# ArthurBrussee/brush

Hardware: NVIDIA H100
Metric: fwd+bwd Mpix/s @1M Gaussians 1080p (higher is better)
Workload: dtype f32

## Files before the change

### brush_b200/csrc/blend_bwd.cu

```cuda
#include "blend_common.cuh"

namespace bg {

constexpr int BROW_ID = 12;
constexpr int BFACT = 12;

__device__ __forceinline__ float rcp_approx_f(float x) { float r; asm("rcp.approx.ftz.f32 %0, %1;" : "=f"(r) : "f"(x)); return r; }
__device__ __forceinline__ float sqrt_approx_f(float x) { float r; asm("sqrt.approx.ftz.f32 %0, %1;" : "=f"(r) : "f"(x)); return r; }

template <bool STATS, bool SMOOTH, bool DEPTH>
__global__ void __launch_bounds__(RASTER_THREADS)
blend_bwd_kernel(const float *__restrict__ projected, const uint32_t *__restrict__ cgid_from_isect,
                 const uint32_t *__restrict__ tile_offsets, const float4 *__restrict__ out_img,
                 const float4 *__restrict__ v_output, const uint32_t *__restrict__ live_masks,
                 const uint32_t *__restrict__ warp_batches, float *__restrict__ v_combined,
                 unsigned long long *__restrict__ stats, BlendUniforms u, const float *__restrict__ depths,
                 const float *__restrict__ out_depth, const float *__restrict__ v_depth, float *__restrict__ v_z) {
    __shared__ BlendStage s_stage[RASTER_WARPS];
    __shared__ __align__(16) float s_fact[RASTER_WARPS][2][WB * BFACT];

    const uint32_t tile = blockIdx.x;
    const uint32_t tid = threadIdx.x, lane = tid & 31u, wid = tid >> 5;
    const uint32_t num_batches = __ldg(warp_batches + tile * RASTER_WARPS + wid);
    BlendStage &st = s_stage[wid];
    if (lane == 0) { mbar_init(&st.bar[0], 1); mbar_init(&st.bar[1], 1); }
    __syncthreads();
    if (num_batches == 0) return;
    uint32_t phase_bits = 0u;
    const uint32_t range_lo = tile_offsets[tile * 2];
    const uint32_t tile_x0 = (tile % u.tiles_x) * TILE_W, tile_y0 = (tile / u.tiles_x) * TILE_W;
    const uint32_t blk_x0 = tile_x0 + 8u * (wid & 1u), blk_y0 = tile_y0 + 8u * (wid >> 1);
    const uint32_t pix_x = blk_x0 + (lane & 7u), pix_y0 = blk_y0 + (lane >> 3), pix_y1 = pix_y0 + 4u;
    const bool inside0 = pix_x < u.img_w && pix_y0 < u.img_h;
    const bool inside1 = pix_x < u.img_w && pix_y1 < u.img_h;
    const float px = (float)pix_x + 0.5f, py0 = (float)pix_y0 + 0.5f;
    const float2 npy2 = make_float2(-py0, -(py0 + 4.0f));
    const float img_wf = (float)u.img_w, img_hf = (float)u.img_h;
    const float hw = img_hf / img_wf, hw2 = hw * hw;

    float2 T2 = make_float2(0.0f, 0.0f);
    float2 rem_r = T2, rem_g = T2, rem_b = T2;
    float2 vo_r = T2, vo_g = T2, vo_b = T2, nvo_w = T2, ifa = T2;
    {
        auto load = [&](bool inside, uint32_t pix_y, float &T, float &rr, float &rg, float &rb, float &vr, float &vg,
                        float &vb, float &nvw, float &inv) {
            if (!inside) return;
            const size_t pix_id = (size_t)pix_x + (size_t)pix_y * u.img_w;
            const float4 o = __ldg(out_img + pix_id);
            const float4 vo = __ldg(v_output + pix_id);
            const float t_final = 1.0f - o.w;
            T = 1.0f;
            rr = o.x - t_final * u.bg_r; rg = o.y - t_final * u.bg_g; rb = o.z - t_final * u.bg_b;
            vr = vo.x; vg = vo.y; vb = vo.z;
            nvw = -((vo.w - (u.bg_r * vo.x + u.bg_g * vo.y + u.bg_b * vo.z)) * t_final);
            inv = img_wf / fmaxf(o.w, 1.0e-5f);
        };
        load(inside0, pix_y0, T2.x, rem_r.x, rem_g.x, rem_b.x, vo_r.x, vo_g.x, vo_b.x, nvo_w.x, ifa.x);
        load(inside1, pix_y1, T2.y, rem_r.y, rem_g.y, rem_b.y, vo_r.y, vo_g.y, vo_b.y, nvo_w.y, ifa.y);
    }
    float2 rem_d = make_float2(0.0f, 0.0f), vo_d = rem_d;
    if constexpr (DEPTH) {
        const size_t pix0 = (size_t)pix_x + (size_t)pix_y0 * u.img_w, pix1 = (size_t)pix_x + (size_t)pix_y1 * u.img_w;
        if (inside0) { rem_d.x = __ldg(out_depth + pix0); vo_d.x = __ldg(v_depth + pix0); }
        if (inside1) { rem_d.y = __ldg(out_depth + pix1); vo_d.y = __ldg(v_depth + pix1); }
    }

    constexpr int NS = DEPTH ? 12 : 10, NH = NS / 2;
    const bool b4 = lane & 16u, b3 = lane & 8u, b2 = lane & 4u, b1 = lane & 2u;
    const uint32_t idx5 = (b3 ? 3u : 0u) + (b2 ? 2u : 0u) + (b1 ? 1u : 0u);
    const uint32_t slot = (b4 ? (uint32_t)NH : 0u) + idx5;
    const bool owner = !(lane & 1u) && !(b2 && b1) && (DEPTH ? slot != 11u : !(b3 && b2));
    const uint32_t lt_mask = (1u << lane) - 1u;

    const size_t mbase = blend_mask_base(range_lo, tile) + wid;
    auto load_mask = [&](uint32_t b) -> uint32_t {
        return b < num_batches ? __ldg(live_masks + mbase + (size_t)b * RASTER_WARPS) : 0u;
    };
    float z_next = 0.0f;
    auto stage = [&](uint32_t b, uint32_t m) -> uint32_t {
        uint32_t id = 0;
        const uint32_t n = (uint32_t)__popc(m);
        if (n == 0) return 0u;
        if ((m >> lane) & 1u) {
            id = __ldg(cgid_from_isect + range_lo + b * WB + lane);
            st.ids[b & 1u][__popc(m & lt_mask)] = id;
            if constexpr (DEPTH) z_next = __ldg(depths + id);
        }
        stage_rows_tma(st, b & 1u, n, projected, lane);
        return id;
    };
    unsigned long long st_iter = 0, st_blend = 0, st_stop = 0;
    uint32_t m_cur = load_mask(0), m_next = load_mask(1);
    uint32_t id_next = stage(0, m_cur);
    for (uint32_t b = 0; b < num_batches; b++) {
        const uint32_t m = m_cur, my_id = id_next;
        const float my_z = z_next;
        m_cur = m_next;
        m_next = load_mask(b + 2);
        id_next = stage(b + 1, m_cur);
        const uint32_t n = (uint32_t)__popc(m);
        if (n == 0) continue;
        mbar_wait(&st.bar[b & 1u], (phase_bits >> (b & 1u)) & 1u);
        phase_bits ^= 1u << (b & 1u);
        float *rows = st.rows[b & 1u];
        float *fact = s_fact[wid][b & 1u];
        if ((m >> lane) & 1u) {
            const uint32_t slot_r = (uint32_t)__popc(m & lt_mask);
            float *mine = rows + slot_r * ROW;
            const float4 B = *reinterpret_cast<const float4 *>(mine + 4);
            const float bcol = mine[8];
            *reinterpret_cast<float4 *>(mine + 4) = make_float4(B.x, -B.y, fmaxf(B.z, 0.0f), fmaxf(B.w, 0.0f));
            mine[8] = fmaxf(bcol, 0.0f);
            mine[BROW_ID] = __uint_as_float(my_id);
            float *f = fact + slot_r * BFACT;
            *reinterpret_cast<float4 *>(f) = make_float4(-1.0f, -1.0f, -0.5f, -1.0f);
            *reinterpret_cast<float4 *>(f + 4) =
                make_float4(-0.5f, B.z >= 0.0f ? -1.0f : 0.0f, B.w >= 0.0f ? -1.0f : 0.0f, bcol >= 0.0f ? -1.0f : 0.0f);
            *reinterpret_cast<float2 *>(f + 8) = make_float2(1.0f / B.y, 1.0f);
            if constexpr (DEPTH) {
                mine[ROW_Z] = my_z;
                *reinterpret_cast<float2 *>(f + 10) = make_float2(-1.0f, 0.0f);
            }
        }
        __syncwarp();
        if (STATS) st_iter += n;
        for (uint32_t j = 0; j < n; j++) {
            const float *row = rows + j * ROW;
            const float4 A = *reinterpret_cast<const float4 *>(row);
            const float4 B = *reinterpret_cast<const float4 *>(row + 4);
            const float4 C = *reinterpret_cast<const float4 *>(row + 8);
            const float dx = A.x - px;
            float2 dy2;
            const float2 sg = pair_sigma(dx, A.y, C.y, C.z, C.w, npy2, dy2);
            const float2 gs = make_float2(ex2_approx(-sg.x), ex2_approx(-sg.y));
            const float2 noa = fmul2_rn(gs, bcast2(B.y));
            const float2 nal = make_float2(fmaxf(-0.999f, noa.x), fmaxf(-0.999f, noa.y));
            float2 nae = nal;
            bool act0, act1;
            if constexpr (SMOOTH) {
                const float2 ae = smooth_alpha(make_float2(-nal.x, -nal.y), sg, act0, act1);
                nae = make_float2(-ae.x, -ae.y);
            } else {
                act0 = sg.x >= 0.0f && noa.x <= -ALPHA_CUTOFF_MID; act1 = sg.y >= 0.0f && noa.y <= -ALPHA_CUTOFF_MID;
            }
            const float2 oma = fadd2_rn(nae, bcast2(1.0f));
            const float2 nT = fmul2_rn(T2, oma);
            const bool c0 = act0 && nT.x > 1.0e-4f, c1 = act1 && nT.y > 1.0e-4f;
            if (STATS) {
                st_blend += __popc(__ballot_sync(0xffffffffu, c0)) + __popc(__ballot_sync(0xffffffffu, c1));
                st_stop += __popc(__ballot_sync(0xffffffffu, act0 && !c0 && T2.x > 1.0e-4f)) +
                           __popc(__ballot_sync(0xffffffffu, act1 && !c1 && T2.y > 1.0e-4f));
            }
            const float2 nalc = make_float2(c0 ? nae.x : 0.0f, c1 ? nae.y : 0.0f);
            const float2 nals = make_float2((c0 && noa.x >= -0.999f) ? nal.x : 0.0f, (c1 && noa.y >= -0.999f) ? nal.y : 0.0f);
            const float2 ra = make_float2(rcp_approx_f(oma.x), rcp_approx_f(oma.y));
            const float2 nvis = fmul2_rn(nalc, T2);
            const float2 G5 = fmul2_rn(nvis, vo_r), G6 = fmul2_rn(nvis, vo_g), G7 = fmul2_rn(nvis, vo_b);
            const float2 u_r = ffma2_rn(T2, bcast2(-B.z), rem_r);
            const float2 u_g = ffma2_rn(T2, bcast2(-B.w), rem_g);
            const float2 u_b = ffma2_rn(T2, bcast2(-C.x), rem_b);
            float2 nd = fmul2_rn(u_r, vo_r);
            nd = ffma2_rn(u_g, vo_g, nd);
            nd = ffma2_rn(u_b, vo_b, nd);
            float z = 0.0f;
            if constexpr (DEPTH) {
                z = row[ROW_Z];
                const float2 u_d = ffma2_rn(T2, bcast2(-z), rem_d);
                nd = ffma2_rn(u_d, vo_d, nd);
            }
            float2 nva = fmul2_rn(fadd2_rn(nd, nvo_w), ra);
            if constexpr (SMOOTH) nva = fmul2_rn(nva, make_float2(smooth_alpha_deriv(-nal.x), smooth_alpha_deriv(-nal.y)));
            const float2 nvs = fmul2_rn(nals, nva);
            const float2 vsx = fmul2_rn(nvs, bcast2(dx)), vsy = fmul2_rn(nvs, dy2);
            const float2 G0 = ffma2_rn(bcast2(A.z), vsx, fmul2_rn(bcast2(A.w), vsy));
            const float2 G1 = ffma2_rn(bcast2(A.w), vsx, fmul2_rn(bcast2(B.x), vsy));
            const float2 G2 = fmul2_rn(vsx, bcast2(dx)), G3 = fmul2_rn(vsx, dy2), G4 = fmul2_rn(vsy, dy2);
            const float2 nn = ffma2_rn(G0, G0, fmul2_rn(fmul2_rn(G1, bcast2(hw2)), G1));
            const float2 G9 = fmul2_rn(make_float2(sqrt_approx_f(nn.x), sqrt_approx_f(nn.y)), ifa);
            rem_r = ffma2_rn(nvis, bcast2(B.z), rem_r);
            rem_g = ffma2_rn(nvis, bcast2(B.w), rem_g);
            rem_b = ffma2_rn(nvis, bcast2(C.x), rem_b);
            float2 G10 = make_float2(0.0f, 0.0f);
            if constexpr (DEPTH) {
                G10 = fmul2_rn(nvis, vo_d);
                rem_d = ffma2_rn(nvis, bcast2(z), rem_d);
            }
            T2.x = act0 ? nT.x : T2.x;
            T2.y = act1 ? nT.y : T2.y;
            float g[NS];
            g[0] = G0.x + G0.y; g[1] = G1.x + G1.y; g[2] = G2.x + G2.y; g[3] = G3.x + G3.y; g[4] = G4.x + G4.y;
            g[5] = G5.x + G5.y; g[6] = G6.x + G6.y; g[7] = G7.x + G7.y; g[8] = nvs.x + nvs.y; g[9] = G9.x + G9.y;
            if constexpr (DEPTH) { g[10] = G10.x + G10.y; g[11] = 0.0f; }
            float a5[6];
#pragma unroll
            for (int i = 0; i < NH; i++) {
                float send = b4 ? g[i] : g[i + NH];
                float keep = b4 ? g[i + NH] : g[i];
                a5[i] = keep + __shfl_xor_sync(0xffffffffu, send, 16);
            }
            if constexpr (!DEPTH) a5[5] = 0.0f;
            float b3v[4];
#pragma unroll
            for (int i = 0; i < 3; i++) {
                float send = b3 ? a5[i] : a5[i + 3];
                float keep = b3 ? a5[i + 3] : a5[i];
                b3v[i] = keep + __shfl_xor_sync(0xffffffffu, send, 8);
            }
            b3v[3] = 0.0f;
            float c2[2];
#pragma unroll
            for (int i = 0; i < 2; i++) {
                float send = b2 ? b3v[i] : b3v[i + 2];
                float keep = b2 ? b3v[i + 2] : b3v[i];
                c2[i] = keep + __shfl_xor_sync(0xffffffffu, send, 4);
            }
            float d1;
            {
                float send = b1 ? c2[0] : c2[1];
                float keep = b1 ? c2[1] : c2[0];
                d1 = keep + __shfl_xor_sync(0xffffffffu, send, 2);
            }
            d1 += __shfl_xor_sync(0xffffffffu, d1, 1);
            if (owner && d1 != 0.0f) {
                const uint32_t id = __float_as_uint(row[BROW_ID]);
                if (DEPTH && slot == 10u) atomicAdd(v_z + id, d1 * fact[j * BFACT + slot]);
                else atomicAdd(v_combined + (size_t)id * BG_VCOMBINED_STRIDE + slot, d1 * fact[j * BFACT + slot]);
            }
        }
        __syncwarp();
    }
    if (STATS && lane == 0) {
        atomicAdd(stats + 0, st_iter); atomicAdd(stats + 1, st_blend); atomicAdd(stats + 2, st_stop);
    }
}

cudaError_t launch_blend_bwd(cudaStream_t s, bool smooth, uint32_t num_tiles, const float *projected, const uint32_t *cgid_from_isect,
                             const uint32_t *tile_offsets, const float *out_img, const float *v_output, const uint32_t *live_masks,
                             const uint32_t *warp_batches, float *v_combined, unsigned long long *stats, uint32_t tiles_x,
                             uint32_t w, uint32_t h, const float *bg, const float *depths, const float *out_depth,
                             const float *v_depth, float *v_z) {
    BlendUniforms u;
    u.tiles_x = tiles_x; u.img_w = w; u.img_h = h; u.bg_r = bg[0]; u.bg_g = bg[1]; u.bg_b = bg[2];
#define BG_LAUNCH_BWD(ST, S, D, STATS_PTR)                                                                                \
    blend_bwd_kernel<ST, S, D><<<num_tiles, RASTER_THREADS, 0, s>>>(projected, cgid_from_isect, tile_offsets, (const float4 *)out_img, \
                                                                    (const float4 *)v_output, live_masks, warp_batches, v_combined, \
                                                                    STATS_PTR, u, depths, out_depth, v_depth, v_z)
    if (v_z) {
        if (smooth) BG_LAUNCH_BWD(false, true, true, nullptr);
        else BG_LAUNCH_BWD(false, false, true, nullptr);
    } else if (smooth) {
        BG_LAUNCH_BWD(false, true, false, nullptr);
    } else if (stats) {
        BG_LAUNCH_BWD(true, false, false, stats);
    } else {
        BG_LAUNCH_BWD(false, false, false, nullptr);
    }
#undef BG_LAUNCH_BWD
    return cudaGetLastError();
}

}
```

### brush_b200/csrc/blend_common.cuh

```cuda
#pragma once
#include "bg_common.cuh"

namespace bg {

constexpr int RASTER_WARPS = 4;
constexpr int RASTER_THREADS = RASTER_WARPS * 32;
constexpr int WB = 32;
constexpr int ROW = BG_PROJECTED_STRIDE;
constexpr int ROW_PT = 12;
constexpr int ROW_Z = 13;

struct BlendUniforms {
    uint32_t tiles_x, img_w, img_h;
    float bg_r, bg_g, bg_b;
};

__device__ __forceinline__ float2 bcast2(float a) { return make_float2(a, a); }

__device__ __forceinline__ size_t blend_mask_base(uint32_t range_lo, uint32_t tile) {
    return ((size_t)(range_lo >> 5) + tile) * RASTER_WARPS;
}

struct __align__(128) BlendStage {
    float rows[2][WB * ROW];
    uint32_t ids[2][WB];
    unsigned long long bar[2];
};

__device__ __forceinline__ void stage_rows_tma(BlendStage &st, uint32_t buf, uint32_t count, const float *projected, uint32_t lane) {
    asm volatile("fence.proxy.async.shared::cta;" ::: "memory");
    __syncwarp();
    if (lane == 0 && count > 0) {
        mbar_expect_tx(&st.bar[buf], count * (ROW * 4u));
        for (uint32_t r = 0; r < count; r++)
            tma_bulk_g2s(&st.rows[buf][r * ROW], projected + (size_t)st.ids[buf][r] * ROW, ROW * 4u, &st.bar[buf]);
    }
}

__device__ __forceinline__ bool block_may_hit(float mx, float my, float a, float b, float c, float thr, float x0,
                                              float x1, float y0, float y1) {
    if (!(a > 0.0f && c > 0.0f && a * c > b * b)) return true;
    const float xc = fminf(fmaxf(mx, x0), x1);
    const float yc = fminf(fmaxf(my, y0), y1);
    const bool out_x = xc != mx, out_y = yc != my;
    if (!(out_x || out_y)) return true;
    float best = 3.0e38f, err = 0.0f;
    if (out_x) {
        float dx = xc - mx;
        float ys = fminf(fmaxf(my - (b / c) * dx, y0), y1);
        float dy = ys - my;
        float t0 = a * dx * dx, t1 = c * dy * dy, t2 = b * dx * dy;
        float s = 0.5f * (t0 + t1) + t2;
        if (s < best) { best = s; err = fabsf(t0) + fabsf(t1) + 2.0f * fabsf(t2); }
    }
    if (out_y) {
        float dy = yc - my;
        float xs = fminf(fmaxf(mx - (b / a) * dy, x0), x1);
        float dx = xs - mx;
        float t0 = a * dx * dx, t1 = c * dy * dy, t2 = b * dx * dy;
        float s = 0.5f * (t0 + t1) + t2;
        if (s < best) { best = s; err = fabsf(t0) + fabsf(t1) + 2.0f * fabsf(t2); }
    }
    return !(best > thr + 0.05f + 4.0e-6f * err);
}

__device__ __forceinline__ float ex2_approx(float x) { float r; asm("ex2.approx.ftz.f32 %0, %1;" : "=f"(r) : "f"(x)); return r; }

__device__ __forceinline__ float2 pair_sigma(float dx, float my, float cy, float cz, float cw, float2 npy2, float2 &dy2) {
    const float hx = __fmul_rn(__fmul_rn(cz, dx), dx);
    const float bdx = __fmul_rn(cw, dx);
    dy2 = fadd2_rn(bcast2(my), npy2);
    float2 t = fmul2_rn(bcast2(cy), dy2);
    t = ffma2_rn(t, dy2, bcast2(hx));
    return ffma2_rn(bcast2(bdx), dy2, t);
}

__device__ __forceinline__ float cutoff_weight(float alpha) {
    const float lo = ALPHA_CUTOFF_MID - 0.5f * ALPHA_CUTOFF_BAND;
    const float t = fminf(fmaxf(__fdiv_rn(__fsub_rn(alpha, lo), ALPHA_CUTOFF_BAND), 0.0f), 1.0f);
    return __fmul_rn(__fmul_rn(t, t), __fmaf_rn(-2.0f, t, 3.0f));
}
__device__ __forceinline__ float cutoff_weight_deriv(float alpha) {
    const float low = ALPHA_CUTOFF_MID - 0.5f * ALPHA_CUTOFF_BAND, high = ALPHA_CUTOFF_MID + 0.5f * ALPHA_CUTOFF_BAND;
    bool inside = alpha > low && alpha < high;
    float t = (alpha - low) / ALPHA_CUTOFF_BAND;
    return inside ? (6.0f * t - 6.0f * t * t) / ALPHA_CUTOFF_BAND : 0.0f;
}
constexpr float SMOOTH_THR_EXTRA = 0.1365f;

__device__ __forceinline__ float2 smooth_alpha(float2 alpha, float2 sg, bool &act0, bool &act1) {
    const float2 w = make_float2(cutoff_weight(alpha.x), cutoff_weight(alpha.y));
    act0 = sg.x >= 0.0f && w.x > 0.0f;
    act1 = sg.y >= 0.0f && w.y > 0.0f;
    return fmul2_rn(alpha, w);
}
__device__ __forceinline__ float smooth_alpha_deriv(float alpha) {
    return fmaf(alpha, cutoff_weight_deriv(alpha), cutoff_weight(alpha));
}

}
```

### brush_b200/csrc/blend_fwd.cu

```cuda
#include "blend_common.cuh"

namespace bg {

template <bool BWD_INFO, bool SMOOTH, bool DEPTH>
__global__ void __launch_bounds__(RASTER_THREADS)
blend_fwd_kernel(const float *__restrict__ projected, const uint32_t *__restrict__ cgid_from_isect,
                 uint32_t *__restrict__ tile_offsets, const uint32_t *__restrict__ gid_from_cgid,
                 float4 *__restrict__ out_f32, uint32_t *__restrict__ out_packed, float *__restrict__ visible,
                 uint32_t *__restrict__ live_masks, uint32_t *__restrict__ warp_batches, BlendUniforms u,
                 const float *__restrict__ depths, float *__restrict__ out_depth) {
    __shared__ BlendStage s_stage[RASTER_WARPS];
    __shared__ uint32_t s_max_useful;

    const uint32_t tile = blockIdx.x;
    const uint32_t tid = threadIdx.x, lane = tid & 31u, wid = tid >> 5;
    const uint32_t tile_x0 = (tile % u.tiles_x) * TILE_W, tile_y0 = (tile / u.tiles_x) * TILE_W;
    const uint32_t blk_x0 = tile_x0 + 8u * (wid & 1u), blk_y0 = tile_y0 + 8u * (wid >> 1);
    const uint32_t pix_x = blk_x0 + (lane & 7u), pix_y0 = blk_y0 + (lane >> 3), pix_y1 = pix_y0 + 4u;
    const bool inside0 = pix_x < u.img_w && pix_y0 < u.img_h;
    const bool inside1 = pix_x < u.img_w && pix_y1 < u.img_h;
    const float px = (float)pix_x + 0.5f, py0 = (float)pix_y0 + 0.5f;
    const float2 npy2 = make_float2(-py0, -(py0 + 4.0f));
    const float rx0 = (float)blk_x0 + 0.5f, rx1 = rx0 + 7.0f, ry0 = (float)blk_y0 + 0.5f, ry1 = ry0 + 7.0f;

    const uint32_t range_lo = tile_offsets[tile * 2], range_hi = tile_offsets[tile * 2 + 1];
    if (BWD_INFO && tid == 0) s_max_useful = range_lo;
    BlendStage &st = s_stage[wid];
    if (lane == 0) { mbar_init(&st.bar[0], 1); mbar_init(&st.bar[1], 1); }
    __syncthreads();
    uint32_t phase_bits = 0u;

    float2 T2 = make_float2(1.0f, 1.0f);
    float2 Tt2 = make_float2(inside0 ? 1.0f : 0.0f, inside1 ? 1.0f : 0.0f);
    float2 r2 = make_float2(0.0f, 0.0f), g2 = r2, b2 = r2, d2 = r2;
    uint32_t last_useful = range_lo;

    const uint32_t num_batches = (range_hi - range_lo + WB - 1) / WB;
    const size_t mbase = blend_mask_base(range_lo, tile) + wid;
    uint32_t batches_walked = 0;
    uint32_t next_id = 0;
    float next_z = 0.0f;
    auto prefetch = [&](uint32_t b) {
        const uint32_t start = range_lo + b * WB;
        const uint32_t count = min((uint32_t)WB, range_hi - start);
        const uint32_t id = lane < count ? __ldg(cgid_from_isect + start + lane) : 0u;
        next_id = id;
        if constexpr (DEPTH) next_z = lane < count ? __ldg(depths + id) : 0.0f;
        if (lane < count) st.ids[b & 1u][lane] = id;
        stage_rows_tma(st, b & 1u, count, projected, lane);
    };
    if (num_batches > 0 && __any_sync(0xffffffffu, inside0 || inside1)) {
        prefetch(0);
        for (uint32_t b = 0; b < num_batches; b++) {
            const uint32_t batch_start = range_lo + b * WB;
            const uint32_t count = min((uint32_t)WB, range_hi - batch_start);
            const uint32_t my_id = next_id;
            const float my_z = next_z;
            if (b + 1 < num_batches) prefetch(b + 1);
            mbar_wait(&st.bar[b & 1u], (phase_bits >> (b & 1u)) & 1u);
            phase_bits ^= 1u << (b & 1u);
            float *rows = st.rows[b & 1u];
            bool hit = false;
            if (lane < count) {
                float *mine = rows + lane * ROW;
                const float4 A = *reinterpret_cast<const float4 *>(mine);
                const float4 B = *reinterpret_cast<const float4 *>(mine + 4);
                const float bcol = mine[8];
                float pt = mine[ROW_PT];
                if constexpr (SMOOTH) pt += SMOOTH_THR_EXTRA;
                hit = block_may_hit(A.x, A.y, A.z, A.w, B.x, pt, rx0, rx1, ry0, ry1);
                *reinterpret_cast<float2 *>(mine + 6) = make_float2(fmaxf(B.z, 0.0f), fmaxf(B.w, 0.0f));
                mine[8] = fmaxf(bcol, 0.0f);
                if constexpr (DEPTH) mine[ROW_Z] = my_z;
            }
            uint32_t bits = __ballot_sync(0xffffffffu, hit);
            uint32_t used_m = 0, acted_m = 0;
            while (bits) {
                const uint32_t s = (uint32_t)__ffs(bits) - 1u;
                bits &= bits - 1u;
                const float *row = rows + s * ROW;
                const float4 A = *reinterpret_cast<const float4 *>(row);
                const float4 B = *reinterpret_cast<const float4 *>(row + 4);
                const float4 C = *reinterpret_cast<const float4 *>(row + 8);
                float2 dy2;
                const float2 sg = pair_sigma(A.x - px, A.y, C.y, C.z, C.w, npy2, dy2);
                const float2 gs = make_float2(ex2_approx(-sg.x), ex2_approx(-sg.y));
                const float2 oa = fmul2_rn(gs, bcast2(B.y));
                float a0 = fminf(0.999f, oa.x), a1 = fminf(0.999f, oa.y);
                bool act0, act1;
                if constexpr (SMOOTH) {
                    const float2 ae = smooth_alpha(make_float2(a0, a1), sg, act0, act1);
                    a0 = ae.x; a1 = ae.y;
                } else {
                    act0 = sg.x >= 0.0f && oa.x >= ALPHA_CUTOFF_MID; act1 = sg.y >= 0.0f && oa.y >= ALPHA_CUTOFF_MID;
                }
                const float2 nT = fmul2_rn(Tt2, fadd2_rn(make_float2(-a0, -a1), bcast2(1.0f)));
                const bool c0 = act0 && nT.x > 1.0e-4f, c1 = act1 && nT.y > 1.0e-4f;
                const float2 vis = fmul2_rn(make_float2(c0 ? a0 : 0.0f, c1 ? a1 : 0.0f), T2);
                r2 = ffma2_rn(bcast2(B.z), vis, r2);
                g2 = ffma2_rn(bcast2(B.w), vis, g2);
                b2 = ffma2_rn(bcast2(C.x), vis, b2);
                if constexpr (DEPTH) d2 = ffma2_rn(bcast2(row[ROW_Z]), vis, d2);
                const uint32_t bit = 1u << s;
                const bool acted = (Tt2.x > 1.0e-4f && act0) || (Tt2.y > 1.0e-4f && act1);
                if (c0 || c1) used_m |= bit;
                if (BWD_INFO && acted) acted_m |= bit;
                T2.x = c0 ? nT.x : T2.x;
                T2.y = c1 ? nT.y : T2.y;
                Tt2.x = act0 ? nT.x : Tt2.x;
                Tt2.y = act1 ? nT.y : Tt2.y;
            }
            const uint32_t used = __reduce_or_sync(0xffffffffu, used_m);
            if (BWD_INFO) {
                const uint32_t acted = __reduce_or_sync(0xffffffffu, acted_m);
                if (lane == 0) live_masks[mbase + (size_t)b * RASTER_WARPS] = acted;
                if ((used >> lane) & 1u) {
                    visible[__ldg(gid_from_cgid + my_id)] = 1.0f;
                    last_useful = batch_start + lane + 1;
                }
            }
            batches_walked = b + 1;
            if (__all_sync(0xffffffffu, !(Tt2.x > 1.0e-4f) && !(Tt2.y > 1.0e-4f))) {
                if (b + 1 < num_batches) mbar_wait(&st.bar[(b + 1) & 1u], (phase_bits >> ((b + 1) & 1u)) & 1u);
                break;
            }
            __syncwarp();
        }
    }

    auto write_pixel = [&](float T, float r, float g, float bl, float d, uint32_t pix_y) {
        const float fr = r + T * u.bg_r, fg = g + T * u.bg_g, fb = bl + T * u.bg_b, fa = 1.0f - T;
        const size_t pix_id = (size_t)pix_x + (size_t)pix_y * u.img_w;
        if (BWD_INFO) {
            out_f32[pix_id] = make_float4(fr, fg, fb, fa);
            if constexpr (DEPTH) out_depth[pix_id] = d;
        } else {
            uint32_t r8 = (uint32_t)fminf(fmaxf(fr * 255.0f, 0.0f), 255.0f);
            uint32_t g8 = (uint32_t)fminf(fmaxf(fg * 255.0f, 0.0f), 255.0f);
            uint32_t b8 = (uint32_t)fminf(fmaxf(fb * 255.0f, 0.0f), 255.0f);
            uint32_t a8 = (uint32_t)fminf(fmaxf(fa * 255.0f, 0.0f), 255.0f);
            out_packed[pix_id] = r8 | (g8 << 8) | (b8 << 16) | (a8 << 24);
        }
    };
    if (inside0) write_pixel(T2.x, r2.x, g2.x, b2.x, d2.x, pix_y0);
    if (inside1) write_pixel(T2.y, r2.y, g2.y, b2.y, d2.y, pix_y1);
    if (BWD_INFO) {
        if (lane == 0) warp_batches[tile * RASTER_WARPS + wid] = batches_walked;
        uint32_t m = last_useful;
        for (int o = 16; o > 0; o >>= 1) m = max(m, __shfl_xor_sync(0xffffffffu, m, o));
        __syncthreads();
        if (lane == 0 && m > range_lo) atomicMax(&s_max_useful, m);
        __syncthreads();
        if (tid == 0) tile_offsets[tile * 2 + 1] = s_max_useful;
    }
}

cudaError_t launch_blend_fwd(cudaStream_t s, bool bwd_info, bool smooth, uint32_t num_tiles, const float *projected,
                             const uint32_t *cgid_from_isect, uint32_t *tile_offsets, const uint32_t *gid_from_cgid, void *out_img,
                             float *visible, uint32_t *live_masks, uint32_t *warp_batches, uint32_t tiles_x, uint32_t w,
                             uint32_t h, const float *bg, const float *depths, float *out_depth) {
    BlendUniforms u;
    u.tiles_x = tiles_x; u.img_w = w; u.img_h = h; u.bg_r = bg[0]; u.bg_g = bg[1]; u.bg_b = bg[2];
#define BG_LAUNCH_FWD(B, S, D, F32, PACKED, LM, WBAT)                                                                    \
    blend_fwd_kernel<B, S, D><<<num_tiles, RASTER_THREADS, 0, s>>>(projected, cgid_from_isect, tile_offsets, gid_from_cgid, \
                                                                   F32, PACKED, visible, LM, WBAT, u, depths, out_depth)
    if (!bwd_info)
        BG_LAUNCH_FWD(false, false, false, nullptr, (uint32_t *)out_img, nullptr, nullptr);
    else if (out_depth && !smooth)
        BG_LAUNCH_FWD(true, false, true, (float4 *)out_img, nullptr, live_masks, warp_batches);
    else if (out_depth)
        BG_LAUNCH_FWD(true, true, true, (float4 *)out_img, nullptr, live_masks, warp_batches);
    else if (!smooth)
        BG_LAUNCH_FWD(true, false, false, (float4 *)out_img, nullptr, live_masks, warp_batches);
    else
        BG_LAUNCH_FWD(true, true, false, (float4 *)out_img, nullptr, live_masks, warp_batches);
#undef BG_LAUNCH_FWD
    return cudaGetLastError();
}

}
```

Measured before the change: 1049.

## Cull splats before TMA staging in forward blend and compact staged rows

The forward blend prefetch now reads each candidate's conic and threshold straight from global memory and runs the block-hit test before staging. Only splats that may hit the block are bulk-copied into shared memory, in compacted order, and the blend loop walks them densely. Used and acted masks are remapped from compact slots back to lane bits with a ballot. This cuts TMA traffic and shared-memory use for culled splats, at the cost of extra global loads per lane during prefetch and extra ballot work. The staging helper is also shared with the backward kernel.

```diff
diff --git a/brush_b200/csrc/blend_bwd.cu b/brush_b200/csrc/blend_bwd.cu
--- a/brush_b200/csrc/blend_bwd.cu
+++ b/brush_b200/csrc/blend_bwd.cu
@@ -79,14 +79,11 @@
     float z_next = 0.0f;
     auto stage = [&](uint32_t b, uint32_t m) -> uint32_t {
         uint32_t id = 0;
-        const uint32_t n = (uint32_t)__popc(m);
-        if (n == 0) return 0u;
         if ((m >> lane) & 1u) {
             id = __ldg(cgid_from_isect + range_lo + b * WB + lane);
-            st.ids[b & 1u][__popc(m & lt_mask)] = id;
             if constexpr (DEPTH) z_next = __ldg(depths + id);
         }
-        stage_rows_tma(st, b & 1u, n, projected, lane);
+        stage_rows_compact(st, b & 1u, m, id, projected, lane);
         return id;
     };
     unsigned long long st_iter = 0, st_blend = 0, st_stop = 0;
diff --git a/brush_b200/csrc/blend_common.cuh b/brush_b200/csrc/blend_common.cuh
--- a/brush_b200/csrc/blend_common.cuh
+++ b/brush_b200/csrc/blend_common.cuh
@@ -35,6 +35,17 @@
         for (uint32_t r = 0; r < count; r++)
             tma_bulk_g2s(&st.rows[buf][r * ROW], projected + (size_t)st.ids[buf][r] * ROW, ROW * 4u, &st.bar[buf]);
     }
+}
+
+__device__ __forceinline__ uint32_t compact_slot(uint32_t m, uint32_t lane) { return (uint32_t)__popc(m & ((1u << lane) - 1u)); }
+
+__device__ __forceinline__ uint32_t stage_rows_compact(BlendStage &st, uint32_t buf, uint32_t m, uint32_t id,
+                                                       const float *projected, uint32_t lane) {
+    const uint32_t n = (uint32_t)__popc(m);
+    if (n == 0) return 0u;
+    if ((m >> lane) & 1u) st.ids[buf][compact_slot(m, lane)] = id;
+    stage_rows_tma(st, buf, n, projected, lane);
+    return n;
 }
 
 __device__ __forceinline__ bool block_may_hit(float mx, float my, float a, float b, float c, float thr, float x0,
diff --git a/brush_b200/csrc/blend_fwd.cu b/brush_b200/csrc/blend_fwd.cu
--- a/brush_b200/csrc/blend_fwd.cu
+++ b/brush_b200/csrc/blend_fwd.cu
@@ -38,81 +38,93 @@
     const uint32_t num_batches = (range_hi - range_lo + WB - 1) / WB;
     const size_t mbase = blend_mask_base(range_lo, tile) + wid;
     uint32_t batches_walked = 0;
-    uint32_t next_id = 0;
+    uint32_t next_id = 0, next_m = 0;
     float next_z = 0.0f;
     auto prefetch = [&](uint32_t b) {
         const uint32_t start = range_lo + b * WB;
-        const uint32_t count = min((uint32_t)WB, range_hi - start);
-        const uint32_t id = lane < count ? __ldg(cgid_from_isect + start + lane) : 0u;
+        const bool in = lane < min((uint32_t)WB, range_hi - start);
+        const uint32_t id = in ? __ldg(cgid_from_isect + start + lane) : 0u;
+        bool cand = false;
+        if (in) {
+            const float4 *row = reinterpret_cast<const float4 *>(projected + (size_t)id * ROW);
+            const float4 A = __ldg(row);
+            const float c = __ldg(projected + (size_t)id * ROW + 4);
+            float pt = __ldg(projected + (size_t)id * ROW + ROW_PT);
+            if constexpr (SMOOTH) pt += SMOOTH_THR_EXTRA;
+            cand = block_may_hit(A.x, A.y, A.z, A.w, c, pt, rx0, rx1, ry0, ry1);
+        }
         next_id = id;
-        if constexpr (DEPTH) next_z = lane < count ? __ldg(depths + id) : 0.0f;
-        if (lane < count) st.ids[b & 1u][lane] = id;
-        stage_rows_tma(st, b & 1u, count, projected, lane);
+        next_m = __ballot_sync(0xffffffffu, cand);
+        if constexpr (DEPTH) next_z = cand ? __ldg(depths + id) : 0.0f;
+        stage_rows_compact(st, b & 1u, next_m, id, projected, lane);
     };
     if (num_batches > 0 && __any_sync(0xffffffffu, inside0 || inside1)) {
         prefetch(0);
         for (uint32_t b = 0; b < num_batches; b++) {
             const uint32_t batch_start = range_lo + b * WB;
-            const uint32_t count = min((uint32_t)WB, range_hi - batch_start);
-            const uint32_t my_id = next_id;
+            const uint32_t m = next_m, my_id = next_id;
             const float my_z = next_z;
+            const uint32_t n = (uint32_t)__popc(m);
             if (b + 1 < num_batches) prefetch(b + 1);
-            mbar_wait(&st.bar[b & 1u], (phase_bits >> (b & 1u)) & 1u);
-            phase_bits ^= 1u << (b & 1u);
-            float *rows = st.rows[b & 1u];
-            bool hit = false;
-            if (lane < count) {
-                float *mine = rows + lane * ROW;
-                const float4 A = *reinterpret_cast<const float4 *>(mine);
-                const float4 B = *reinterpret_cast<const float4 *>(mine + 4);
-                const float bcol = mine[8];
-                float pt = mine[ROW_PT];
-                if constexpr (SMOOTH) pt += SMOOTH_THR_EXTRA;
-                hit = block_may_hit(A.x, A.y, A.z, A.w, B.x, pt, rx0, rx1, ry0, ry1);
-                *reinterpret_cast<float2 *>(mine + 6) = make_float2(fmaxf(B.z, 0.0f), fmaxf(B.w, 0.0f));
-                mine[8] = fmaxf(bcol, 0.0f);
-                if constexpr (DEPTH) mine[ROW_Z] = my_z;
+            else next_m = 0u;
+            uint32_t used = 0, acted = 0;
+            if (n > 0) {
+                mbar_wait(&st.bar[b & 1u], (phase_bits >> (b & 1u)) & 1u);
+                phase_bits ^= 1u << (b & 1u);
+                float *rows = st.rows[b & 1u];
+                if ((m >> lane) & 1u) {
+                    float *mine = rows + compact_slot(m, lane) * ROW;
+                    const float4 B = *reinterpret_cast<const float4 *>(mine + 4);
+                    const float bcol = mine[8];
+                    *reinterpret_cast<float2 *>(mine + 6) = make_float2(fmaxf(B.z, 0.0f), fmaxf(B.w, 0.0f));
+                    mine[8] = fmaxf(bcol, 0.0f);
+                    if constexpr (DEPTH) mine[ROW_Z] = my_z;
+                }
+                __syncwarp();
+                uint32_t used_m = 0, acted_m = 0;
+                for (uint32_t j = 0; j < n; j++) {
+                    const float *row = rows + j * ROW;
+                    const float4 A = *reinterpret_cast<const float4 *>(row);
+                    const float4 B = *reinterpret_cast<const float4 *>(row + 4);
+                    const float4 C = *reinterpret_cast<const float4 *>(row + 8);
+                    float2 dy2;
+                    const float2 sg = pair_sigma(A.x - px, A.y, C.y, C.z, C.w, npy2, dy2);
+                    const float2 gs = make_float2(ex2_approx(-sg.x), ex2_approx(-sg.y));
+                    const float2 oa = fmul2_rn(gs, bcast2(B.y));
+                    float a0 = fminf(0.999f, oa.x), a1 = fminf(0.999f, oa.y);
+                    bool act0, act1;
+                    if constexpr (SMOOTH) {
+                        const float2 ae = smooth_alpha(make_float2(a0, a1), sg, act0, act1);
+                        a0 = ae.x; a1 = ae.y;
+                    } else {
+                        act0 = sg.x >= 0.0f && oa.x >= ALPHA_CUTOFF_MID; act1 = sg.y >= 0.0f && oa.y >= ALPHA_CUTOFF_MID;
+                    }
+                    const float2 nT = fmul2_rn(Tt2, fadd2_rn(make_float2(-a0, -a1), bcast2(1.0f)));
+                    const bool c0 = act0 && nT.x > 1.0e-4f, c1 = act1 && nT.y > 1.0e-4f;
+                    const float2 vis = fmul2_rn(make_float2(c0 ? a0 : 0.0f, c1 ? a1 : 0.0f), T2);
+                    r2 = ffma2_rn(bcast2(B.z), vis, r2);
+                    g2 = ffma2_rn(bcast2(B.w), vis, g2);
+                    b2 = ffma2_rn(bcast2(C.x), vis, b2);
+                    if constexpr (DEPTH) d2 = ffma2_rn(bcast2(row[ROW_Z]), vis, d2);
+                    const uint32_t bit = 1u << j;
+                    const bool acts = (Tt2.x > 1.0e-4f && act0) || (Tt2.y > 1.0e-4f && act1);
+                    if (c0 || c1) used_m |= bit;
+                    if (BWD_INFO && acts) acted_m |= bit;
+                    T2.x = c0 ? nT.x : T2.x;
+                    T2.y = c1 ? nT.y : T2.y;
+                    Tt2.x = act0 ? nT.x : Tt2.x;
+                    Tt2.y = act1 ? nT.y : Tt2.y;
+                }
+                const bool cand = (m >> lane) & 1u;
+                const uint32_t slot = compact_slot(m, lane);
+                const uint32_t used_c = __reduce_or_sync(0xffffffffu, used_m);
+                used = __ballot_sync(0xffffffffu, cand && ((used_c >> slot) & 1u));
+                if (BWD_INFO) {
+                    const uint32_t acted_c = __reduce_or_sync(0xffffffffu, acted_m);
+                    acted = __ballot_sync(0xffffffffu, cand && ((acted_c >> slot) & 1u));
+                }
             }
-            uint32_t bits = __ballot_sync(0xffffffffu, hit);
-            uint32_t used_m = 0, acted_m = 0;
-            while (bits) {
-                const uint32_t s = (uint32_t)__ffs(bits) - 1u;
-                bits &= bits - 1u;
-                const float *row = rows + s * ROW;
-                const float4 A = *reinterpret_cast<const float4 *>(row);
-                const float4 B = *reinterpret_cast<const float4 *>(row + 4);
-                const float4 C = *reinterpret_cast<const float4 *>(row + 8);
-                float2 dy2;
-                const float2 sg = pair_sigma(A.x - px, A.y, C.y, C.z, C.w, npy2, dy2);
-                const float2 gs = make_float2(ex2_approx(-sg.x), ex2_approx(-sg.y));
-                const float2 oa = fmul2_rn(gs, bcast2(B.y));
-                float a0 = fminf(0.999f, oa.x), a1 = fminf(0.999f, oa.y);
-                bool act0, act1;
-                if constexpr (SMOOTH) {
-                    const float2 ae = smooth_alpha(make_float2(a0, a1), sg, act0, act1);
-                    a0 = ae.x; a1 = ae.y;
-                } else {
-                    act0 = sg.x >= 0.0f && oa.x >= ALPHA_CUTOFF_MID; act1 = sg.y >= 0.0f && oa.y >= ALPHA_CUTOFF_MID;
-                }
-                const float2 nT = fmul2_rn(Tt2, fadd2_rn(make_float2(-a0, -a1), bcast2(1.0f)));
-                const bool c0 = act0 && nT.x > 1.0e-4f, c1 = act1 && nT.y > 1.0e-4f;
-                const float2 vis = fmul2_rn(make_float2(c0 ? a0 : 0.0f, c1 ? a1 : 0.0f), T2);
-                r2 = ffma2_rn(bcast2(B.z), vis, r2);
-                g2 = ffma2_rn(bcast2(B.w), vis, g2);
-                b2 = ffma2_rn(bcast2(C.x), vis, b2);
-                if constexpr (DEPTH) d2 = ffma2_rn(bcast2(row[ROW_Z]), vis, d2);
-                const uint32_t bit = 1u << s;
-                const bool acted = (Tt2.x > 1.0e-4f && act0) || (Tt2.y > 1.0e-4f && act1);
-                if (c0 || c1) used_m |= bit;
-                if (BWD_INFO && acted) acted_m |= bit;
-                T2.x = c0 ? nT.x : T2.x;
-                T2.y = c1 ? nT.y : T2.y;
-                Tt2.x = act0 ? nT.x : Tt2.x;
-                Tt2.y = act1 ? nT.y : Tt2.y;
-            }
-            const uint32_t used = __reduce_or_sync(0xffffffffu, used_m);
             if (BWD_INFO) {
-                const uint32_t acted = __reduce_or_sync(0xffffffffu, acted_m);
                 if (lane == 0) live_masks[mbase + (size_t)b * RASTER_WARPS] = acted;
                 if ((used >> lane) & 1u) {
                     visible[__ldg(gid_from_cgid + my_id)] = 1.0f;
@@ -120,8 +132,8 @@
                 }
             }
             batches_walked = b + 1;
-            if (__all_sync(0xffffffffu, !(Tt2.x > 1.0e-4f) && !(Tt2.y > 1.0e-4f))) {
-                if (b + 1 < num_batches) mbar_wait(&st.bar[(b + 1) & 1u], (phase_bits >> ((b + 1) & 1u)) & 1u);
+            if (n > 0 && __all_sync(0xffffffffu, !(Tt2.x > 1.0e-4f) && !(Tt2.y > 1.0e-4f))) {
+                if (next_m != 0u) mbar_wait(&st.bar[(b + 1) & 1u], (phase_bits >> ((b + 1) & 1u)) & 1u);
                 break;
             }
             __syncwarp();
```

New measurement: 1055 (median of 6 runs). Within noise of the previous version (+0.5%).
